# electronicarts/mesh2splat

Measured on AMD Instinct MI355X. Metric: Gaussians/sec emitted (mesh->3DGS conversion pass, density 1024^2), higher is better.
Workload: dtype f32

## Files before the change

include/m2s.h:

```cpp
#ifndef M2S_H
#define M2S_H

#include <stddef.h>
#include <stdint.h>

#ifdef __cplusplus
extern "C" {
#endif

#define M2S_ABI_VERSION 1

typedef enum m2s_status {
    M2S_OK = 0,
    M2S_ERR_INVALID = 1,
    M2S_ERR_NO_DEVICE = 2,
    M2S_ERR_HIP = 3,
    M2S_ERR_OOM = 4,
    M2S_ERR_CAPACITY = 5,
    M2S_ERR_IO = 6,
    M2S_ERR_STATE = 7
} m2s_status;

typedef struct m2s_ctx m2s_ctx;

// ... 290 lines not shown
uint32_t m2s_host_scene_num_meshes(const m2s_host_scene* scene);
const m2s_mesh* m2s_host_scene_meshes(const m2s_host_scene* scene);
const char* m2s_host_scene_mesh_name(const m2s_host_scene* scene, uint32_t i);
const char* m2s_host_scene_warnings(const m2s_host_scene* scene);
m2s_status m2s_read_ply(const char* path, m2s_gaussian** out_records, uint64_t* out_n, int* out_has_pbr);
void m2s_free_records(m2s_gaussian* records);
const char* m2s_io_last_error(void);

enum { M2S_PIPELINE_AUTO = 0, M2S_PIPELINE_MULTIPASS = 1,
       M2S_PIPELINE_TEAM = 3 ,
       M2S_PIPELINE_SPARSE = 4 ,
       M2S_PIPELINE_LEAN = 5  };
m2s_status m2s_set_pipeline(m2s_ctx* ctx, int pipeline);
int m2s_last_pipeline(const m2s_ctx* ctx);
m2s_status m2s_vertex_table(const m2s_ctx* ctx, uint64_t* out_rows, int* out_in_use);

enum { M2S_K_COUNT = 0, M2S_K_SCAN = 1, M2S_K_OFFSETS = 2, M2S_K_EMIT = 3, M2S_K_FUSED = 4, M2S_K_N = 5 };
m2s_status m2s_set_profiling(m2s_ctx* ctx, int enabled);
m2s_status m2s_last_kernel_ms(const m2s_ctx* ctx, float out_ms[M2S_K_N]);
uint64_t m2s_num_triangles(const m2s_ctx* ctx);
m2s_status m2s_debug_set_launch_counter(m2s_ctx* ctx, uint32_t value);

#ifdef __cplusplus
}
#endif
#endif
```

mesh2splat_amd/_lib.py:

```python
from __future__ import annotations

import ctypes as C
import os
import subprocess

_HERE = os.path.dirname(os.path.abspath(__file__))
CSRC = os.path.join(_HERE, "csrc")
LIB_PATH = os.environ.get("M2S_LIB_PATH") or os.path.join(_HERE, "_build", "libm2s_hip.so")

M2S_OK = 0
STATUS_NAMES = {0: "M2S_OK", 1: "M2S_ERR_INVALID", 2: "M2S_ERR_NO_DEVICE", 3: "M2S_ERR_HIP", 4: "M2S_ERR_OOM",
                5: "M2S_ERR_CAPACITY", 6: "M2S_ERR_IO", 7: "M2S_ERR_STATE"}
KERNEL_NAMES = ("count", "scan", "offsets", "emit", "fused")

EXPORTS = (
    "m2s_abi_version", "m2s_create", "m2s_destroy", "m2s_last_error", "m2s_set_triangle_range", "m2s_upload_scene",
    "m2s_set_max_gaussians", "m2s_convert", "m2s_convert_into", "m2s_convert_submit", "m2s_convert_wait", "m2s_last_pipeline", "m2s_set_keep_positions", "m2s_positions_ready", "m2s_debug_set_launch_counter", "m2s_set_async_lanes", "m2s_num_stored", "m2s_device_records", "m2s_download",
    "m2s_download_triangle_counts", "m2s_write_ply", "m2s_export_ply", "m2s_set_profiling", "m2s_last_kernel_ms",
    "m2s_num_triangles", "m2s_set_pipeline", "m2s_load_glb", "m2s_free_host_scene", "m2s_host_scene_num_meshes",
    "m2s_host_scene_meshes", "m2s_host_scene_mesh_name", "m2s_host_scene_warnings", "m2s_read_ply", "m2s_free_records",
    "m2s_io_last_error", "m2s_sort_by_depth", "m2s_device_sorted_records", "m2s_download_sorted", "m2s_last_sort_ms",
    "m2s_upload_records", "m2s_prepass", "m2s_device_quads", "m2s_device_prepass_depths", "m2s_download_prepass", "m2s_last_prepass_ms",
    "m2s_sort_prepass", "m2s_prepass_sorted", "m2s_device_sorted_quads", "m2s_download_sorted_quads", "m2s_last_sort_prepass_ms",
    "m2s_last_upload_ms", "m2s_write_ply_slice", "m2s_export_ply_slice",
# ... 6 lines not shown
    "m2s_last_splat_counts",
    "m2s_shadow", "m2s_shadow_from_quads", "m2s_device_shadow_cubemap", "m2s_download_shadow_cubemap", "m2s_download_shadow_quads", "m2s_upload_shadow_cubemap",
    "m2s_last_shadow_ms", "m2s_last_shadow_stage_ms", "m2s_last_shadow_counts", "m2s_relight", "m2s_upload_gbuffer", "m2s_device_frame",
    "m2s_download_frame", "m2s_download_shadow_counts", "m2s_last_relight_ms",
    "m2s_mesh_depth", "m2s_device_mesh_depth", "m2s_download_mesh_depth", "m2s_last_mesh_depth_ms", "m2s_last_mesh_depth_stage_ms",
    "m2s_last_mesh_depth_counts", "m2s_debug_set_mesh_depth_inplace",
    "m2s_mesh_render", "m2s_device_mesh_gbuffer", "m2s_download_mesh_gbuffer", "m2s_download_mesh_visibility", "m2s_last_mesh_render_ms",
    "m2s_last_mesh_render_stage_ms", "m2s_last_mesh_render_counts", "m2s_relight_split",
    "m2s_relight_mesh", "m2s_device_mesh_frame", "m2s_download_mesh_frame", "m2s_score_frames", "m2s_device_score_map",
    "m2s_download_score_map", "m2s_last_score_ms",
    "m2s_bake_light", "m2s_bake_directions", "m2s_device_sh", "m2s_download_sh", "m2s_download_bake_shadow_counts", "m2s_last_bake_ms",
    "m2s_sh_shade_records", "m2s_write_ply_sh", "m2s_export_ply_sh",
    "m2s_device_sorted_sources", "m2s_download_sorted_sources", "m2s_upload_quad_sources", "m2s_contrib_begin", "m2s_contrib_accumulate", "m2s_device_contrib",
    "m2s_download_contrib", "m2s_last_contrib_ms", "m2s_last_contrib_stage_ms", "m2s_prune", "m2s_last_prune_counts", "m2s_last_prune_ms",
    "m2s_write_ply_compact", "m2s_export_ply_compact", "m2s_last_compact_stage_ms",
    "m2s_vertex_table",
)


class M2SError(RuntimeError):
    def __init__(self, status: int, message: str):
        super().__init__(f"{STATUS_NAMES.get(status, status)}: {message}")
        self.status = status


class Texture(C.Structure):
    _fields_ = [("rgba8", C.c_void_p), ("width", C.c_uint32), ("height", C.c_uint32)]


class MeshC(C.Structure):
    _fields_ = [("vertices", C.c_void_p), ("n_vertices", C.c_uint32), ("stride_floats", C.c_uint32),
# ... 176 lines not shown
        "m2s_download_sorted_sources": (C.c_int, [vp, vp, u64]),
        "m2s_upload_quad_sources": (C.c_int, [vp, vp, u64]),
        "m2s_contrib_begin": (C.c_int, [vp]),
        "m2s_contrib_accumulate": (C.c_int, [vp, vp, C.c_float]),
        "m2s_device_contrib": (vp, [vp, u32]),
        "m2s_download_contrib": (C.c_int, [vp, vp, vp, u64]),
        "m2s_last_contrib_ms": (C.c_float, [vp]),
        "m2s_last_contrib_stage_ms": (C.c_int, [vp, C.POINTER(C.c_float)]),
        "m2s_prune": (C.c_int, [vp, vp, C.POINTER(u64)]),
        "m2s_last_prune_counts": (C.c_int, [vp, C.POINTER(u64)]),
        "m2s_last_prune_ms": (C.c_float, [vp]),
        "m2s_write_ply_compact": (C.c_int, [C.c_char_p, vp, vp, u32, u64, C.c_float, C.POINTER(u64)]),
        "m2s_export_ply_compact": (C.c_int, [vp, C.c_char_p, C.c_float, C.c_int, C.POINTER(u64)]),
        "m2s_last_compact_stage_ms": (C.c_int, [vp, C.POINTER(C.c_float)]),
        "m2s_vertex_table": (C.c_int, [vp, C.POINTER(u64), C.POINTER(C.c_int)]),
    }
    for name, (res, args) in sigs.items():
        fn = getattr(L, name)
        fn.restype = res
        fn.argtypes = args
    _lib = L
    return L
```

mesh2splat_amd/converter.py:

```python
from __future__ import annotations

import ctypes as C
import os
from typing import Optional

import numpy as np

from . import _lib
from .scene import RECORD_FLOATS, TEXTURE_SLOTS, Scene


def marshal_scene(scene: Scene):
    n = scene.n_meshes
    arr = (_lib.MeshC * max(1, n))()
    keep = []
    for i, m in enumerate(scene.meshes):
        v = np.ascontiguousarray(m.vertices, np.float32)
        keep.append(v)
        arr[i].vertices = v.ctypes.data
        arr[i].n_vertices = v.shape[0]
        arr[i].stride_floats = v.shape[1]
        for k in range(3):
            arr[i].bbox_min[k] = float(m.bbox_min[k])
            arr[i].bbox_max[k] = float(m.bbox_max[k])
# ... 754 lines not shown
    def set_pipeline(self, name: str):
        self._check(self._L.m2s_set_pipeline(self._h, {"auto": 0, "multipass": 1, "team": 3, "sparse": 4, "lean": 5}[name]))

    def set_async_lanes(self, lanes: int):
        self._check(self._L.m2s_set_async_lanes(self._h, int(lanes)))

    @property
    def last_pipeline(self) -> str:
        return {0: "none", 1: "multipass", 3: "team", 4: "sparse", 5: "lean"}[self._L.m2s_last_pipeline(self._h)]

    def vertex_table(self) -> dict:
        rows, used = C.c_uint64(0), C.c_int(0)
        self._check(self._L.m2s_vertex_table(self._h, C.byref(rows), C.byref(used)))
        return {"rows": int(rows.value), "in_use": bool(used.value)}

    def set_profiling(self, on: bool):
        self._check(self._L.m2s_set_profiling(self._h, 1 if on else 0))

    def last_kernel_ms(self) -> dict:
        ms = (C.c_float * len(_lib.KERNEL_NAMES))()
        self._check(self._L.m2s_last_kernel_ms(self._h, ms))
        return {k: float(ms[i]) for i, k in enumerate(_lib.KERNEL_NAMES)}


def write_ply(path: str, records: np.ndarray, fmt: int, scale_multiplier: float):
    r = np.ascontiguousarray(records, np.float32)
    if r.ndim != 2 or r.shape[1] != RECORD_FLOATS:
        raise ValueError("records must be (n, 24) float32")
    st = _lib.load().m2s_write_ply(os.fsencode(path), r.ctypes.data, r.shape[0], int(fmt), float(scale_multiplier))
    if st != _lib.M2S_OK:
# ... 140 lines not shown
```

mesh2splat_amd/csrc/m2s_context.cpp:

```cpp
#include "m2s_ctx.h"

#include <algorithm>
#include <chrono>
#include <cstring>
#include <string>

using namespace m2s;
using namespace m2s_host;

namespace {
thread_local std::string g_create_error = "";
}

namespace m2s_host {
void free_scene(m2s_ctx* c) {
    c->tri_mem.release(); c->scene_arena.release();
    c->lane[0].release_scene(false); c->lane[1].release_scene(true);
    c->d_meshes = nullptr; c->d_mesh_first = nullptr;
    c->d_cnt = c->d_partials = nullptr;
    c->d_biglist = nullptr; c->d_bigmeta = nullptr; c->d_bands = nullptr; c->run_table_words = 0; c->d_run_order = nullptr; c->run_order_unit = 0;
    c->d_batch_first = nullptr; c->n_batch_tab = 0; c->chain_words = 0;
    c->rinfo.clear();
    ++c->rinfo_gen;
    c->frag_per_R2 = -1.0;
    c->warm_R = 0; c->warm_total = 0; c->warm_mismatch_seen = false;
    c->sparse_off_R = c->team_off_R = c->lean_off_R = UINT32_MAX;
    c->lean_ok = false;
    c->d_vt_rows.release(); c->d_vt_ids.release();
    c->vt_rows = 0; c->vt_use = false;
    c->scene = SceneDev{};
    c->has_scene = false;
}

m2s_ctx::RInfo& rinfo_for(m2s_ctx* c, uint32_t R) {
    auto it = c->rinfo.find(R);
    if (it != c->rinfo.end()) return it->second;
    if (c->rinfo.size() >= (size_t)kBandSlots) { drain_in_flight(c); c->rinfo.clear(); ++c->rinfo_gen; }
    m2s_ctx::RInfo ri;
    ri.gen = c->rinfo_gen;
    ri.band_slot = (int)c->rinfo.size();
    return c->rinfo.emplace(R, ri).first->second;
}

static bool spin_waits() { static const bool on = !debug_on("M2S_NO_SPIN"); return on; }
// ... 130 lines not shown
        ++c->rinfo_gen;
    }
    c->pipeline = pipeline;
    return M2S_OK;
}

int m2s_last_pipeline(const m2s_ctx* c) { return c ? c->last_pipeline : 0; }

m2s_status m2s_vertex_table(const m2s_ctx* c, uint64_t* out_rows, int* out_in_use) {
    if (!c) return M2S_ERR_INVALID;
    if (out_rows) *out_rows = c->vt_rows;
    if (out_in_use) *out_in_use = c->vt_use ? 1 : 0;
    return M2S_OK;
}

int m2s_positions_ready(const m2s_ctx* c) {
    return c && c->d_pos_plane && c->last_records && c->pos_plane_of == c->last_records && c->pos_plane_n == c->last_stored &&
           c->pos_plane_epoch == c->records_epoch && c->last_stored ? 1 : 0;
}

m2s_status m2s_set_keep_positions(m2s_ctx* c, int enabled) {
    if (!c) return M2S_ERR_INVALID;
    c->keep_positions = enabled != 0;
    return M2S_OK;
}

m2s_status m2s_debug_set_launch_counter(m2s_ctx* c, uint32_t value) {
    if (!c) return M2S_ERR_INVALID;
    if (c->slot_count) return fail(c, M2S_ERR_STATE, kInFlightMsg);
    c->epoch = value;
// ... 19 lines not shown
```

mesh2splat_amd/csrc/m2s_ctx.h:

```cpp
#pragma once
#include "../../include/m2s.h"
#include "m2s_devbuf.h"
#include "m2s_device.h"
#include "m2s_vdedup.h"

#include <cstdint>
#include <cstdlib>
#include <map>
#include <string>

namespace m2s_host {
constexpr uint32_t kMaxGaussiansToSort = 7000000u;
constexpr uint64_t kMaxTriangles = (1ull << 28) - 1;
inline size_t align_up(size_t v, size_t a) { return (v + a - 1) / a * a; }
inline const char* const kStaleMsg = "the records of the conversion last waited for have been overwritten by a later submission at another R "
                                     "(wait for it, or submit into your own buffers)";
inline const char* const kInFlightMsg = "conversions are still in flight: m2s_convert_wait first";
struct GBufPlanes {
    DevBuf<void> plane[5];
    void* ptr[5] = {};
    m2s_status reserve(std::string& err, uint64_t px) {
        for (int k = 0; k < 5; ++k) {
            const m2s_status s = plane[k].reserve(err, px, (k == 2 || k == 4) ? 4 : 8);
            ptr[k] = plane[k].get();
// ... 11 lines not shown
    hipStream_t stream = nullptr;
    std::string err;

    m2s_host::DevBuf<char> tri_mem;
    m2s::SceneDev scene{};
    m2s::MeshParams* d_meshes = nullptr;
    uint32_t* d_mesh_first = nullptr;
    uint32_t n_meshes_total = 0;
    bool has_scene = false;
    bool lean_ok = false;
    uint64_t range_first = 0, range_count = UINT64_MAX;
    m2s_host::DevBuf<float4> d_vt_rows;
    m2s_host::DevBuf<m2s::VtIds> d_vt_ids;
    uint32_t vt_rows = 0;
    bool vt_use = false;

    uint32_t* d_cnt = nullptr;
    uint32_t* d_partials = nullptr;
    m2s_host::PinnedBuf<unsigned long long> h_total;
    static constexpr int kPinnedPrepass = 2 + 2 * M2S_MAX_IN_FLIGHT;
    static constexpr int kPinnedSortMM = 4 + 2 * M2S_MAX_IN_FLIGHT;
    static constexpr int kPinnedWords = 6 + 2 * M2S_MAX_IN_FLIGHT;
    m2s::BigItem* d_biglist = nullptr;
    uint32_t* d_bigmeta = nullptr;
    struct RInfo {
        int form = M2S_PIPELINE_AUTO;
        uint32_t tpw = 0;
        bool async_ok = false;
        bool mp_ready = false;
        bool bands_ready = false;
// ... 236 lines not shown
```

mesh2splat_amd/csrc/m2s_devfn.h:

```cpp
#pragma once
#include "m2s_device.h"
#include "m2s_exact.h"
#include "m2s_vtable.h"

#pragma clang fp contract(off)

namespace m2s {

__device__ __forceinline__ float len3(float x, float y, float z) { return sqrtf((x * x + y * y) + z * z); }
__device__ __forceinline__ float len3sq(float x, float y, float z) { return (x * x + y * y) + z * z; }
__device__ __forceinline__ float inv_len3(float x, float y, float z) {
    const float q = len3sq(x, y, z);
    if (wave_all(in_sqrt_range(q))) return rcp_rn(sqrt_rn(q));
    return 1.0f / sqrtf(q);
}

__device__ __forceinline__ uint32_t wave_incl_scan(uint32_t v, int ) {
    v += (uint32_t)__builtin_amdgcn_update_dpp(0, (int)v, 0x111, 0xf, 0xf, true);
    v += (uint32_t)__builtin_amdgcn_update_dpp(0, (int)v, 0x112, 0xf, 0xf, true);
    v += (uint32_t)__builtin_amdgcn_update_dpp(0, (int)v, 0x114, 0xf, 0xf, true);
    v += (uint32_t)__builtin_amdgcn_update_dpp(0, (int)v, 0x118, 0xf, 0xf, true);
    v += (uint32_t)__builtin_amdgcn_update_dpp(0, (int)v, 0x142, 0xa, 0xf, true);
    v += (uint32_t)__builtin_amdgcn_update_dpp(0, (int)v, 0x143, 0xc, 0xf, true);
    return v;
// ... 576 lines not shown
    float4 rot;
    uint32_t vid_lo, vid_hi;
    uint32_t org;
    uint32_t mesh;
};
static_assert(sizeof(TriShadeSI) == 64, "TriShadeSI must be four float4");
template <class TS> inline constexpr bool kTsHasIds = false;
template <> inline constexpr bool kTsHasIds<TriShadeSI> = true;

__device__ __forceinline__ float lod_from_grad(float fw, float fh, float dudx, float dvdx, float dudy, float dvdy) {
    const float sx = dudx * fw, tx = dvdx * fh, sy = dudy * fw, ty = dvdy * fh;
    const float r2 = fmaxf(fma_(tx, tx, sx * sx), fma_(ty, ty, sy * sy));
    return 0.5f * fast_log2(r2);
}

template <class MP, class TS>
__device__ __forceinline__ void tri_shade_rest(const float p[9], const Geo& g, int a1, int b1, int a2, int b2, MP mp,
                                               float4 b0, float2 b1uv, TS& ts) {
    ts.mesh = 0;
    const float A1 = (float)a1 * 256.0f * ts.inva, B1 = (float)b1 * 256.0f * ts.inva;
    const float A2 = (float)a2 * 256.0f * ts.inva, B2 = (float)b2 * 256.0f * ts.inva;
    geo_flat(p, g, ts.sx, ts.sy, ts.rot);
    ts.lod0 = ts.lod1 = ts.lod2 = 0.0f;
    const auto ta = &mp->tex[0];
    const auto tn = &mp->tex[1];
    const auto tm = &mp->tex[2];
    const bool hasA = ta->texels != nullptr, hasN = tn->texels != nullptr, hasM = tm->texels != nullptr;
    if (hasA || hasN || hasM) {
        const float du1 = b0.z - b0.x, du2 = b1uv.x - b0.x, dv1 = b0.w - b0.y, dv2 = b1uv.y - b0.y;
        const float dudx = fma_(A2, du2, A1 * du1), dvdx = fma_(A2, dv2, A1 * dv1);
        const float dudy = fma_(B2, du2, B1 * du1), dvdy = fma_(B2, dv2, B1 * dv1);
        if (hasA) ts.lod0 = lod_from_grad((float)ta->w, (float)ta->h, dudx, dvdx, dudy, dvdy);
        if (hasN) ts.lod1 = (hasA && tn->w == ta->w && tn->h == ta->h) ? ts.lod0
                          : lod_from_grad((float)tn->w, (float)tn->h, dudx, dvdx, dudy, dvdy);
        if (hasM) ts.lod2 = (hasA && tm->w == ta->w && tm->h == ta->h) ? ts.lod0
                          : (hasN && tm->w == tn->w && tm->h == tn->h) ? ts.lod1
                          : lod_from_grad((float)tm->w, (float)tm->h, dudx, dvdx, dudy, dvdy);
// ... 20 lines not shown
template <class MP>
__device__ __forceinline__ void tri_shade_setup(const float p[9], const Geo& g, const Raster& rs, MP mp,
                                                float4 b0, float2 b1, TriShade& ts) {
    {
#pragma clang fp contract(off)
        ts.inva = rcp_rn((float)rs.area2);
    }
    const long long Px0 = 256ll * rs.x0 + 128, Py0 = 256ll * rs.y0 + 128;
    ts.a1 = rs.a[1]; ts.b1 = rs.b[1]; ts.a2 = rs.a[2]; ts.b2 = rs.b[2];
    ts.e1 = (long long)rs.a[1] * Px0 + (long long)rs.b[1] * Py0 + rs.c[1];
    ts.e2 = (long long)rs.a[2] * Px0 + (long long)rs.b[2] * Py0 + rs.c[2];
    ts.org = ((uint32_t)rs.y0 << 12) | (uint32_t)rs.x0;
    tri_shade_rest(p, g, rs.a[1], rs.b[1], rs.a[2], rs.b[2], mp, b0, b1, ts);
}

template <class MP>
__device__ __forceinline__ void tri_shade_small(const float p[9], const Geo& g, const RasterHead& h, const RasterSmall& rs, MP mp, float4 b0, float2 b1,
                                                uint32_t m, TriShadeS& c) {
    {
#pragma clang fp contract(off)
        c.inva = rcp_rn((float)rs.area2);
    }
    c.a1 = (short)rs.a[1]; c.b1 = (short)rs.b[1]; c.a2 = (short)rs.a[2]; c.b2 = (short)rs.b[2];
    c.e1 = rs.e[1]; c.e2 = rs.e[2];
    c.org = ((uint32_t)h.y0 << 12) | (uint32_t)h.x0;
    tri_shade_rest(p, g, rs.a[1], rs.b[1], rs.a[2], rs.b[2], mp, b0, b1, c);
    c.mesh |= m;
}

struct TexTap {
    uint32_t o00, o10, o01, o11;
    float w00, w10, w01, w11;
};

__device__ __forceinline__ void tex_tap(uint32_t W, uint32_t H, uint32_t level_off, float uf, float vf, TexTap& t) {
    float up, vp;
    {
#pragma clang fp contract(off)
        up = uf * (float)W - 0.5f;
        vp = vf * (float)H - 0.5f;
    }
// ... 321 lines not shown
```

mesh2splat_amd/csrc/m2s_device.h:

```cpp
#pragma once
#include <cstdlib>
#include <hip/hip_runtime.h>
#include <stdint.h>

#include "m2s_vtable.h"

namespace m2s {

#ifdef M2S_DEBUG_BUILD
inline const char* debug_env(const char* name) {
    static const bool enabled = std::getenv("M2S_DEBUG") != nullptr;
    return enabled ? std::getenv(name) : nullptr;
}
#else
inline const char* debug_env(const char*) { return nullptr; }
#endif
inline bool debug_on(const char* name) { const char* v = debug_env(name); return v && *v && *v != '0'; }

constexpr int kBlock = 256;
constexpr int kTriPerBlock = 1024;
constexpr int kEmitF = 1024;
constexpr int kRowsThread = 32;
constexpr int kRowsCount = 128;
constexpr int kStageStride = 7;
// ... 93 lines not shown
    if (const char* v = debug_env("M2S_RUN_SHIFT")) { const uint32_t s = (uint32_t)std::atoi(v) & 15u; return n_units >= (32u << s) ? s : 0u; }
    for (uint32_t shift = 5; shift >= 3; --shift)
        if (n_units >= (32u << shift)) return shift;
    return 0u;
}
inline uint32_t n_runs(uint32_t n_units, uint32_t shift) { return (n_units + (1u << shift) - 1u) >> shift; }
struct BatchTable {
    const uint32_t* first;
    uint32_t n;
    uint32_t tpw;
};
uint32_t fused2_band_workgroups(uint32_t n_tri);
void launch_fused2(const SceneDev& sc, uint32_t R, unsigned long long* chain, uint64_t limit, float4* out,
                   unsigned long long* total, uint32_t* status, uint32_t epoch, BigItem* biglist, uint32_t* bigmeta,
                   const RunInfo& runs, const BatchTable& batches, hipStream_t st);
void launch_fused3(const SceneDev& sc, uint32_t R, unsigned long long* chain, uint64_t limit, float4* out,
                   unsigned long long* total, uint32_t* status, uint32_t epoch, BigItem* biglist, uint32_t* bigmeta,
                   const RunInfo& runs, const BatchTable& batches, hipStream_t st, const VtxTable* vt = nullptr);
void launch_sparse(const SceneDev& sc, uint32_t R, unsigned long long* chain, uint64_t limit, float4* out,
                   unsigned long long* total, uint32_t* status, uint32_t epoch, BigItem* biglist, uint32_t* bigmeta,
                   const RunInfo& runs, hipStream_t st, float4* plane = nullptr);
bool sparse_supported(uint32_t n_tri);
uint32_t sparse_workgroups(uint32_t n_tri);
constexpr uint32_t kSparseTrianglesPerWorkgroup = 512;
void launch_emit_big(const SceneDev& sc, uint32_t R, const BigItem* biglist, uint32_t n_big, uint32_t max_cnt, uint64_t limit,
                     float4* out, hipStream_t st);

struct PrepassK {
    float M[16], V[16], P[16];
    float MinvT[16];
    float mr_inv[9];
    float ms2[3];
    float res[2], near_far[2], std_dev;
// ... 167 lines not shown
```

mesh2splat_amd/csrc/m2s_fused3.hip:

```cpp
#include "m2s_fused_common.h"

#include <type_traits>

#pragma clang fp contract(off)

namespace m2s {

#ifndef M2S_FUSED3_WAVES
#define M2S_FUSED3_WAVES 4
#endif
#ifndef M2S_FUSED3_ENTRIES
#define M2S_FUSED3_ENTRIES 1024
#endif
#ifndef M2S_FUSED3_STAGE
#define M2S_FUSED3_STAGE (M2S_FUSED3_WAVES >= 5 ? 16 : 32)
#endif
constexpr int kL3Team = 4;
constexpr int kL3Threads = kL3Team * 64;
constexpr uint32_t kL3Entries = (uint32_t)M2S_FUSED3_ENTRIES * kL3Team;
constexpr int kL3Stage = M2S_FUSED3_STAGE;
constexpr uint32_t kL3Wait = 1u << 24;
constexpr uint32_t kL3Stop = 1u << 28;

struct F3Ctl {
// ... 76 lines not shown
    return true;
}

#ifdef M2S_TIMELINE
__device__ unsigned long long g_tl_f3[16384 * 4 * 8];
constexpr int kTlHwId = 4 | (31 << 11);
constexpr int kTlXccId = 20 | (3 << 11);
#define TLF(k) do { __builtin_amdgcn_sched_barrier(0); if (lane == 0 && blockIdx.x < 16384u) g_tl_f3[((size_t)blockIdx.x * 4 + wave) * 8 + (k)] = wall_clock64(); __builtin_amdgcn_sched_barrier(0); } while (0)
#define TLFV(k, v) do { if (lane == 0 && blockIdx.x < 16384u) g_tl_f3[((size_t)blockIdx.x * 4 + wave) * 8 + (k)] = (v); } while (0)
#else
#define TLF(k) do { } while (0)
#define TLFV(k, v) do { } while (0)
#endif

struct VtNone { };
template <bool kIndexed>
__global__ void __launch_bounds__(kL3Threads, M2S_FUSED3_WAVES) k_fused3(SceneDev sc, uint32_t R, unsigned long long* __restrict__ chain,
                                                      unsigned long long limit, float4* __restrict__ out,
                                                      unsigned long long* __restrict__ total_out,
                                                      uint32_t* __restrict__ status , uint32_t epoch,
                                                      BigItem* __restrict__ biglist, uint32_t* __restrict__ bigmeta,
                                                      uint32_t tpw ,
                                                      RunInfo runs, BatchTable bt,
                                                      std::conditional_t<kIndexed, VtxTable, VtNone> vt) {
    using TS = std::conditional_t<kIndexed, TriShadeSI, TriShadeS>;
    __shared__ F3Lds S;
    F3Ctl& C = S.ctl;
    const int lane = threadIdx.x & 63;
    const uint32_t wave = __builtin_amdgcn_readfirstlane(threadIdx.x >> 6);
    const uint32_t n_batches = bt.first ? bt.n : (sc.n_tri + tpw - 1u) / tpw;
    const uint32_t hb = blockIdx.x, xcd = hb & 7u, round = hb >> 3;
    const bool in_runs = runs.base != nullptr;
    const uint32_t rmask = (1u << runs.shift) - 1u;
    const unsigned long long etag = (unsigned long long)epoch << kEpochShift;
    uint32_t lb = hb;
    if (in_runs) {
        uint32_t rr = ((round >> runs.shift) << 3) + xcd;
        if (runs.order) rr = ((const __attribute__((address_space(4))) uint32_t*)runs.order)[rr];
        lb = (rr << runs.shift) + (round & rmask);
// ... 25 lines not shown
    const unsigned long long band_base = band_first ? C.base : 0ull;

    uint32_t t0 = b * tpw, nt = tpw;
    if (bt.first && has_batch) {
        const __attribute__((address_space(4))) uint32_t* q = (const __attribute__((address_space(4))) uint32_t*)bt.first;
        t0 = q[b];
        nt = q[b + 1] - t0;
    }
    const uint32_t t = t0 + lane;
    const bool valid = has_batch && (uint32_t)lane < nt && t < sc.n_tri;
    if (lane == 0) C.t0[wave] = t0;
    int kind = kNone;
    unsigned long long mask = 0;
    uint32_t cnt = 0;
    {
        float p[9];
        Geo g;
        RasterHead h;
        h.x0 = h.y0 = 0; h.x1 = h.y1 = -1; h.ext = 0;
        bool box = false;
        uint32_t m = 0;
        float4 uvb0 = make_float4(0, 0, 0, 0);
        float2 uvb1 = make_float2(0, 0);
        [[maybe_unused]] uint2 vid = make_uint2(0, 0);
        bool uniform_mesh = false;
        uint32_t m0 = 0;
        if (has_batch) {
            const uint32_t lastT = min(t0 + nt, sc.n_tri) - 1;
            m0 = mesh_of_range(sc, t0, lastT, uniform_mesh);
            m = m0;
            if (valid) {
                load_positions(sc.tri, t, p);
                uvb0 = sc.tri.B0[t];
                uvb1 = sc.tri.B1[t];
                if constexpr (kIndexed) vid = ld_plane(reinterpret_cast<const uint2*>(vt.ids), t);
                if (uniform_mesh) geo_setup_mp(p, kConstMesh(sc.meshes + m0), g);
                else { m = find_mesh(sc, sc.tri_first + t); geo_setup_mp(p, sc.meshes + m, g); }
                box = raster_head(g, R, h);
            }
        }
        const int w = h.x1 - h.x0 + 1, rows = h.y1 - h.y0 + 1;
        RasterSmall rs;
        bool small = box && w <= 8 && rows <= 8 && h.ext <= 2304;
        if (small) small = raster_small(h, rs);
        else if (box) kind = kBig;
        {
            uint32_t mlo = 0, mhi = 0;
            small_coverage(small, w, rows, rs, mlo, mhi);
            mask = (unsigned long long)mlo | ((unsigned long long)mhi << 32);
            cnt = (uint32_t)__popc(mlo) + (uint32_t)__popc(mhi);
            if (small) kind = kSmall;
        }
        if (cnt != 0 && kind == kSmall) {
            TriShadeS c;
            if (uniform_mesh) tri_shade_small(p, g, h, rs, kConstMesh(sc.meshes + m0), uvb0, uvb1, m, c);
            else tri_shade_small(p, g, h, rs, sc.meshes + m, uvb0, uvb1, m, c);
            const float4* src = reinterpret_cast<const float4*>(&c);
#pragma unroll
            for (int k = 0; k < 3; ++k) S.tri[wave][lane * 4 + k] = src[k];
            if constexpr (kIndexed) S.tri[wave][lane * 4 + 3] = make_float4(__uint_as_float(vid.x), __uint_as_float(vid.y), src[3].z, src[3].w);
            else S.tri[wave][lane * 4 + 3] = src[3];
            float2* const uvs = &S.uv[wave][lane * 3];
            uvs[0] = make_float2(uvb0.x, uvb0.y);
            uvs[1] = make_float2(uvb0.z - uvb0.x, uvb0.w - uvb0.y);
            uvs[2] = make_float2(uvb1.x - uvb0.x, uvb1.y - uvb0.y);
        }
        if (__ballot(kind == kBig) != 0ull) {
            Raster rb;
            rb.x0 = rb.y0 = 0; rb.x1 = rb.y1 = -1; rb.ext = 0; rb.bias = 0; rb.area2 = 1;
#pragma unroll
            for (int i = 0; i < 3; i++) { rb.a[i] = rb.b[i] = 0; rb.c[i] = 0; }
// ... 239 lines not shown
        if (!have_base) have_base = f3_get_base(C, chain, b0, lane, epoch, status, base);
        if (have_base && lane == 0) {
            const unsigned long long out_total = (C.total_w[0] + C.total_w[1]) + (C.total_w[2] + C.total_w[3]);
            chain_store(&chain[b0 + nb_here - 1], kFlagPrefix | etag | ((base + out_total) & kValMask));
            if (b0 + nb_here == n_batches) *total_out = base + out_total;
            if (runs.out && (lb & rmask) == 0u) runs.out[lb >> runs.shift] = base;
        }
    }
    if (err && lane == 0) __hip_atomic_store(&status[1], err, __ATOMIC_RELAXED, __HIP_MEMORY_SCOPE_SYSTEM);
    TLF(5);
    TLFV(7, (unsigned long long)lb | ((unsigned long long)__builtin_amdgcn_s_getreg(kTlHwId) << 32));
}

void launch_fused3(const SceneDev& sc, uint32_t R, unsigned long long* chain, uint64_t limit, float4* out,
                   unsigned long long* total, uint32_t* status, uint32_t epoch, BigItem* biglist, uint32_t* bigmeta,
                   const RunInfo& runs, const BatchTable& bt, hipStream_t st, const VtxTable* vt) {
    const uint32_t tpw = fused_tpw(sc.n_tri);
    const uint32_t n_batches = bt.first ? bt.n : n_fused_waves(sc.n_tri);
    if (!n_batches) return;
    uint32_t nb = (n_batches + kL3Team - 1) / kL3Team;
    RunInfo r = runs;
    if (tpw != 64u || bt.first) r = RunInfo{ nullptr, nullptr, 0u, nullptr };
    if (r.base) r.out = nullptr;
    if (r.base) nb = ((nb + (8u << r.shift) - 1u) / (8u << r.shift)) * (8u << r.shift);
    else nb = (nb + 7u) & ~7u;
    if (vt && vt->rows && vt->ids)
        hipLaunchKernelGGL(k_fused3<true>, dim3(nb), dim3(kL3Threads), 0, st, sc, R, chain, (unsigned long long)limit, out, total, status,
                           epoch & 0xFFFFu, biglist, bigmeta, tpw, r, bt, *vt);
    else
        hipLaunchKernelGGL(k_fused3<false>, dim3(nb), dim3(kL3Threads), 0, st, sc, R, chain, (unsigned long long)limit, out, total, status,
                           epoch & 0xFFFFu, biglist, bigmeta, tpw, r, bt, VtNone{});
}

#ifdef M2S_TIMELINE
}
extern "C" int m2s_debug_timeline_f3(void* dst, size_t bytes) {
    return hipMemcpyFromSymbol(dst, HIP_SYMBOL(m2s::g_tl_f3), std::min(bytes, sizeof(m2s::g_tl_f3))) == hipSuccess ? 0 : 1;
}
extern "C" int m2s_debug_timeline_f3_clear() {
    void* p = nullptr;
    if (hipGetSymbolAddress(&p, HIP_SYMBOL(m2s::g_tl_f3)) != hipSuccess) return 1;
    return hipMemset(p, 0, sizeof(m2s::g_tl_f3)) == hipSuccess ? 0 : 2;
}
namespace m2s {
#endif
uint32_t fused3_resident_workgroups() { return resident_workgroups(reinterpret_cast<const void*>(&k_fused3<false>), kL3Threads); }
hipError_t preload_fused3() { hipFuncAttributes a; return hipFuncGetAttributes(&a, reinterpret_cast<const void*>(&k_fused3<false>)); }

}
```

mesh2splat_amd/csrc/m2s_pass.cpp:

```cpp
#include "m2s_ctx.h"

#include <algorithm>
#include <cstdio>
#include <cstring>
#include <vector>

using namespace m2s;
using namespace m2s_host;

namespace {
static double sparse_frags_per_triangle(uint32_t n_tri) { return n_tri >= 2000000u ? 1.75 : 0.5; }
static uint32_t band_workgroups(const m2s_ctx* c, uint32_t unit) {
    const uint32_t team = fused2_band_workgroups(c->scene.n_tri);
    return !team ? 0u : unit == 256u ? team : sparse_workgroups(c->scene.n_tri);
}
static uint32_t first_resident_slots([[maybe_unused]] int form, [[maybe_unused]] uint32_t shift) {
#ifdef M2S_RUN_ORDER_SPREAD
    const uint32_t wgs = form == M2S_PIPELINE_SPARSE ? sparse_resident_workgroups() : form == M2S_PIPELINE_LEAN ? fused3_resident_workgroups()
                                                                                                                 : fused2_resident_workgroups();
    return wgs >> shift;
#else
    return 0u;
#endif
}
// ... 18 lines not shown
}

BatchTable batches_for(const m2s_ctx* c, const m2s_ctx::RInfo& ri) {
    return c->n_batch_tab ? BatchTable{ c->d_batch_first, c->n_batch_tab, 0u } : BatchTable{ nullptr, 0u, ri.tpw };
}

uint32_t unit_of(int form) { return form == M2S_PIPELINE_SPARSE ? kSparseTrianglesPerWorkgroup : 256u; }

void launch_single(const m2s_ctx* c, const m2s_ctx::RInfo& ri, uint32_t R, unsigned long long* chain, uint64_t limit, float4* d_out,
                   unsigned long long* res, uint32_t epoch, const RunInfo& runs, hipStream_t st, float4* plane) {
    uint32_t* status = reinterpret_cast<uint32_t*>(&res[1]);
    if (ri.form == M2S_PIPELINE_SPARSE)
        launch_sparse(c->scene, R, chain, limit, d_out, &res[0], status, epoch, c->d_biglist, c->d_bigmeta, runs, st, plane);
    else if (ri.form == M2S_PIPELINE_LEAN) {
        const VtxTable vt{ c->d_vt_rows.get(), c->d_vt_ids.get() };
        launch_fused3(c->scene, R, chain, limit, d_out, &res[0], status, epoch, c->d_biglist, c->d_bigmeta, runs, batches_for(c, ri), st,
                      c->vt_use ? &vt : nullptr);
    }
    else
        launch_fused2(c->scene, R, chain, limit, d_out, &res[0], status, epoch, c->d_biglist, c->d_bigmeta, runs, batches_for(c, ri), st);
}

uint64_t resolve_cap(const m2s_ctx* c, uint32_t R) {
    if (c->cap_policy == 0) return 0;
    if (c->cap_policy > 0) return (uint64_t)c->cap_policy;
    const uint32_t mc = std::max<uint32_t>(1u, c->n_meshes_total);
    const uint32_t mx = R * R * 6u * mc;
    return std::min(mx, kMaxGaussiansToSort);
}
}

static bool lean_eligible(const m2s_ctx* c, uint32_t R) {
// ... 402 lines not shown
```

mesh2splat_amd/csrc/m2s_upload.cpp:

```cpp
#include "m2s_ctx.h"
#include "m2s_ply.h"

#include <algorithm>
#include <array>
#include <chrono>
#include <cstring>
#include <thread>
#include <tuple>
#include <vector>

using namespace m2s;
using namespace m2s_host;

namespace {
constexpr size_t kStageChunk = 16ull << 20;

void par_memcpy(void* dst, const void* src, size_t n) {
    const size_t kMin = 2ull << 20;
    unsigned nt = (unsigned)std::min<size_t>(4, n / kMin);
    if (const char* e = std::getenv("M2S_HOST_THREADS")) { if (std::atol(e) == 1) nt = 1; }
    if (nt <= 1) { memcpy(dst, src, n); return; }
    std::vector<std::thread> pool;
    for (unsigned i = 1; i < nt; ++i) {
        const size_t b = n * i / nt, e = n * (i + 1) / nt;
// ... 220 lines not shown
    c->d_batch_first = (uint32_t*)(A + o_batch);
    c->n_batch_tab = 0;
    c->chain_words = chain_words;
    HIPCHK(c, hipMemsetAsync(c->lane[0].chain, 0, chain_words * sizeof(unsigned long long), c->stream));
    HIPCHK(c, hipMemsetAsync(c->d_bigmeta, 0, 4 * sizeof(uint32_t), c->stream));
    const uint32_t warm_R = c->hint_R ? c->hint_R : c->last_R ? c->last_R : 1024u;
    const bool warm = !debug_on("M2S_NO_WARM");
    bool counted = false;
    if (warm && !debug_on("M2S_NO_WARM_OVERLAP")) counted = warm_count_enqueue(c, warm_R) == M2S_OK;
    VtWork vt_work;
    bool vt_begun = false;
    if (vt_size_ok(c->lean_ok, n_tri) && !debug_on("M2S_NO_VTABLE")) {
        vt_begun = vt_dedup_begin(tp, n_tri, vt_work, c->stream) == hipSuccess;
        if (!vt_begun) (void)hipGetLastError();
    }

    for (TexPlan& p : tex_plan) {
        uint32_t* mem = (uint32_t*)(A + p.arena_off);
        const m2s_status st = staged_h2d(c, (const char*)p.src, (size_t)p.d.w * p.d.h * 4, kStageChunk, (char*)mem, turn,
                                         [](char*, size_t, size_t) {});
        if (st != M2S_OK) return st;
        for (uint32_t l = 1; l < p.d.n_levels; ++l)
            launch_mip_level(mem + p.d.off[l - 1], std::max(1u, p.d.w >> (l - 1)), std::max(1u, p.d.h >> (l - 1)),
                             mem + p.d.off[l], std::max(1u, p.d.w >> l), std::max(1u, p.d.h >> l), c->stream);
    }
    for (ComboPlan& cp : combo_plan) {
        uint32_t* mem = (uint32_t*)(A + cp.arena_off);
        const TexDesc &ta = tex_plan[cp.ia].d, &tn = tex_plan[cp.in].d, &tm = tex_plan[cp.im].d;
        for (uint32_t l = 0; l < ta.n_levels; ++l)
            launch_combo_level(ta.texels + ta.off[l], tn.texels + tn.off[l], tm.texels + tm.off[l], std::max(1u, ta.w >> l),
// ... 54 lines not shown
```

Measured before the change: 28.92 billion.

## Precompute per-triangle geometry planes at upload for the lean fused kernel

A new kernel runs at scene upload and computes each triangle's flat-geometry terms (rotation, scales, projected UV offsets), storing them in three float4 planes. The lean fused3 kernel gains a template variant that reads these planes instead of loading positions and running geo_setup and geo_flat on every convert. This moves per-triangle setup work out of the timed conversion pass. In exchange it adds 48 bytes per triangle of device memory and extra loads per triangle in the hot kernel.

```diff
diff --git a/include/m2s.h b/include/m2s.h
--- a/include/m2s.h
+++ b/include/m2s.h
@@ -328,6 +328,7 @@
 m2s_status m2s_set_pipeline(m2s_ctx* ctx, int pipeline);
 int m2s_last_pipeline(const m2s_ctx* ctx);
 m2s_status m2s_vertex_table(const m2s_ctx* ctx, uint64_t* out_rows, int* out_in_use);
+m2s_status m2s_geo_planes(const m2s_ctx* ctx, uint64_t* out_bytes, int* out_in_use);
 
 enum { M2S_K_COUNT = 0, M2S_K_SCAN = 1, M2S_K_OFFSETS = 2, M2S_K_EMIT = 3, M2S_K_FUSED = 4, M2S_K_N = 5 };
 m2s_status m2s_set_profiling(m2s_ctx* ctx, int enabled);
diff --git a/mesh2splat_amd/_lib.py b/mesh2splat_amd/_lib.py
--- a/mesh2splat_amd/_lib.py
+++ b/mesh2splat_amd/_lib.py
@@ -44,7 +44,7 @@
     "m2s_device_sorted_sources", "m2s_download_sorted_sources", "m2s_upload_quad_sources", "m2s_contrib_begin", "m2s_contrib_accumulate", "m2s_device_contrib",
     "m2s_download_contrib", "m2s_last_contrib_ms", "m2s_last_contrib_stage_ms", "m2s_prune", "m2s_last_prune_counts", "m2s_last_prune_ms",
     "m2s_write_ply_compact", "m2s_export_ply_compact", "m2s_last_compact_stage_ms",
-    "m2s_vertex_table",
+    "m2s_vertex_table", "m2s_geo_planes",
 )
 
 
@@ -251,6 +251,7 @@
         "m2s_export_ply_compact": (C.c_int, [vp, C.c_char_p, C.c_float, C.c_int, C.POINTER(u64)]),
         "m2s_last_compact_stage_ms": (C.c_int, [vp, C.POINTER(C.c_float)]),
         "m2s_vertex_table": (C.c_int, [vp, C.POINTER(u64), C.POINTER(C.c_int)]),
+        "m2s_geo_planes": (C.c_int, [vp, C.POINTER(u64), C.POINTER(C.c_int)]),
     }
     for name, (res, args) in sigs.items():
         fn = getattr(L, name)
diff --git a/mesh2splat_amd/converter.py b/mesh2splat_amd/converter.py
--- a/mesh2splat_amd/converter.py
+++ b/mesh2splat_amd/converter.py
@@ -792,6 +792,11 @@
         self._check(self._L.m2s_vertex_table(self._h, C.byref(rows), C.byref(used)))
         return {"rows": int(rows.value), "in_use": bool(used.value)}
 
+    def geo_planes(self) -> dict:
+        nbytes, used = C.c_uint64(0), C.c_int(0)
+        self._check(self._L.m2s_geo_planes(self._h, C.byref(nbytes), C.byref(used)))
+        return {"bytes": int(nbytes.value), "in_use": bool(used.value)}
+
     def set_profiling(self, on: bool):
         self._check(self._L.m2s_set_profiling(self._h, 1 if on else 0))
 
diff --git a/mesh2splat_amd/csrc/m2s_context.cpp b/mesh2splat_amd/csrc/m2s_context.cpp
--- a/mesh2splat_amd/csrc/m2s_context.cpp
+++ b/mesh2splat_amd/csrc/m2s_context.cpp
@@ -28,6 +28,7 @@
     c->lean_ok = false;
     c->d_vt_rows.release(); c->d_vt_ids.release();
     c->vt_rows = 0; c->vt_use = false;
+    c->geo_stride = 0; c->geo_use = false;
     c->scene = SceneDev{};
     c->has_scene = false;
 }
@@ -188,6 +189,13 @@
     return M2S_OK;
 }
 
+m2s_status m2s_geo_planes(const m2s_ctx* c, uint64_t* out_bytes, int* out_in_use) {
+    if (!c) return M2S_ERR_INVALID;
+    if (out_bytes) *out_bytes = c->geo_use ? (uint64_t)c->scene.n_tri * 3u * sizeof(float4) : 0u;
+    if (out_in_use) *out_in_use = c->geo_use ? 1 : 0;
+    return M2S_OK;
+}
+
 int m2s_positions_ready(const m2s_ctx* c) {
     return c && c->d_pos_plane && c->last_records && c->pos_plane_of == c->last_records && c->pos_plane_n == c->last_stored &&
            c->pos_plane_epoch == c->records_epoch && c->last_stored ? 1 : 0;
diff --git a/mesh2splat_amd/csrc/m2s_ctx.h b/mesh2splat_amd/csrc/m2s_ctx.h
--- a/mesh2splat_amd/csrc/m2s_ctx.h
+++ b/mesh2splat_amd/csrc/m2s_ctx.h
@@ -49,6 +49,9 @@
     m2s_host::DevBuf<m2s::VtIds> d_vt_ids;
     uint32_t vt_rows = 0;
     bool vt_use = false;
+    m2s_host::DevBuf<float4> d_geo;
+    size_t geo_stride = 0;
+    bool geo_use = false;
 
     uint32_t* d_cnt = nullptr;
     uint32_t* d_partials = nullptr;
diff --git a/mesh2splat_amd/csrc/m2s_devfn.h b/mesh2splat_amd/csrc/m2s_devfn.h
--- a/mesh2splat_amd/csrc/m2s_devfn.h
+++ b/mesh2splat_amd/csrc/m2s_devfn.h
@@ -614,13 +614,13 @@
     return 0.5f * fast_log2(r2);
 }
 
-template <class MP, class TS>
+template <bool kFlat = true, class MP, class TS>
 __device__ __forceinline__ void tri_shade_rest(const float p[9], const Geo& g, int a1, int b1, int a2, int b2, MP mp,
                                                float4 b0, float2 b1uv, TS& ts) {
     ts.mesh = 0;
     const float A1 = (float)a1 * 256.0f * ts.inva, B1 = (float)b1 * 256.0f * ts.inva;
     const float A2 = (float)a2 * 256.0f * ts.inva, B2 = (float)b2 * 256.0f * ts.inva;
-    geo_flat(p, g, ts.sx, ts.sy, ts.rot);
+    if constexpr (kFlat) geo_flat(p, g, ts.sx, ts.sy, ts.rot);
     ts.lod0 = ts.lod1 = ts.lod2 = 0.0f;
     const auto ta = &mp->tex[0];
     const auto tn = &mp->tex[1];
@@ -671,7 +671,7 @@
     tri_shade_rest(p, g, rs.a[1], rs.b[1], rs.a[2], rs.b[2], mp, b0, b1, ts);
 }
 
-template <class MP>
+template <bool kFlat = true, class MP>
 __device__ __forceinline__ void tri_shade_small(const float p[9], const Geo& g, const RasterHead& h, const RasterSmall& rs, MP mp, float4 b0, float2 b1,
                                                 uint32_t m, TriShadeS& c) {
     {
@@ -681,7 +681,7 @@
     c.a1 = (short)rs.a[1]; c.b1 = (short)rs.b[1]; c.a2 = (short)rs.a[2]; c.b2 = (short)rs.b[2];
     c.e1 = rs.e[1]; c.e2 = rs.e[2];
     c.org = ((uint32_t)h.y0 << 12) | (uint32_t)h.x0;
-    tri_shade_rest(p, g, rs.a[1], rs.b[1], rs.a[2], rs.b[2], mp, b0, b1, c);
+    tri_shade_rest<kFlat>(p, g, rs.a[1], rs.b[1], rs.a[2], rs.b[2], mp, b0, b1, c);
     c.mesh |= m;
 }
 
diff --git a/mesh2splat_amd/csrc/m2s_device.h b/mesh2splat_amd/csrc/m2s_device.h
--- a/mesh2splat_amd/csrc/m2s_device.h
+++ b/mesh2splat_amd/csrc/m2s_device.h
@@ -131,9 +131,16 @@
 void launch_fused2(const SceneDev& sc, uint32_t R, unsigned long long* chain, uint64_t limit, float4* out,
                    unsigned long long* total, uint32_t* status, uint32_t epoch, BigItem* biglist, uint32_t* bigmeta,
                    const RunInfo& runs, const BatchTable& batches, hipStream_t st);
+struct GeoPlanes {
+    const float4* G0;
+    const float4* G1;
+    const float4* G2;
+};
+void launch_geo_planes(const SceneDev& sc, float4* g0, float4* g1, float4* g2, hipStream_t st);
 void launch_fused3(const SceneDev& sc, uint32_t R, unsigned long long* chain, uint64_t limit, float4* out,
                    unsigned long long* total, uint32_t* status, uint32_t epoch, BigItem* biglist, uint32_t* bigmeta,
-                   const RunInfo& runs, const BatchTable& batches, hipStream_t st, const VtxTable* vt = nullptr);
+                   const RunInfo& runs, const BatchTable& batches, hipStream_t st, const VtxTable* vt = nullptr,
+                   const GeoPlanes* gp = nullptr);
 void launch_sparse(const SceneDev& sc, uint32_t R, unsigned long long* chain, uint64_t limit, float4* out,
                    unsigned long long* total, uint32_t* status, uint32_t epoch, BigItem* biglist, uint32_t* bigmeta,
                    const RunInfo& runs, hipStream_t st, float4* plane = nullptr);
diff --git a/mesh2splat_amd/csrc/m2s_fused3.hip b/mesh2splat_amd/csrc/m2s_fused3.hip
--- a/mesh2splat_amd/csrc/m2s_fused3.hip
+++ b/mesh2splat_amd/csrc/m2s_fused3.hip
@@ -114,7 +114,8 @@
 #endif
 
 struct VtNone { };
-template <bool kIndexed>
+struct GeoNone { };
+template <bool kIndexed, bool kGeo>
 __global__ void __launch_bounds__(kL3Threads, M2S_FUSED3_WAVES) k_fused3(SceneDev sc, uint32_t R, unsigned long long* __restrict__ chain,
                                                       unsigned long long limit, float4* __restrict__ out,
                                                       unsigned long long* __restrict__ total_out,
@@ -122,7 +123,8 @@
                                                       BigItem* __restrict__ biglist, uint32_t* __restrict__ bigmeta,
                                                       uint32_t tpw ,
                                                       RunInfo runs, BatchTable bt,
-                                                      std::conditional_t<kIndexed, VtxTable, VtNone> vt) {
+                                                      std::conditional_t<kIndexed, VtxTable, VtNone> vt,
+                                                      std::conditional_t<kGeo, GeoPlanes, GeoNone> gp) {
     using TS = std::conditional_t<kIndexed, TriShadeSI, TriShadeS>;
     __shared__ F3Lds S;
     F3Ctl& C = S.ctl;
@@ -178,8 +180,10 @@
     unsigned long long mask = 0;
     uint32_t cnt = 0;
     {
-        float p[9];
+        [[maybe_unused]] float p[9];
         Geo g;
+        [[maybe_unused]] float4 grot = make_float4(0, 0, 0, 0);
+        [[maybe_unused]] float gsx = 0, gsy = 0;
         RasterHead h;
         h.x0 = h.y0 = 0; h.x1 = h.y1 = -1; h.ext = 0;
         bool box = false;
@@ -194,11 +198,18 @@
             m0 = mesh_of_range(sc, t0, lastT, uniform_mesh);
             m = m0;
             if (valid) {
-                load_positions(sc.tri, t, p);
+                [[maybe_unused]] float4 q0, q1, q2;
+                if constexpr (kGeo) { q0 = ld_plane(gp.G0, t); q1 = ld_plane(gp.G1, t); q2 = ld_plane(gp.G2, t); }
+                else load_positions(sc.tri, t, p);
                 uvb0 = sc.tri.B0[t];
                 uvb1 = sc.tri.B1[t];
                 if constexpr (kIndexed) vid = ld_plane(reinterpret_cast<const uint2*>(vt.ids), t);
-                if (uniform_mesh) geo_setup_mp(p, kConstMesh(sc.meshes + m0), g);
+                if constexpr (kGeo) {
+                    grot = q0; gsx = q1.x; gsy = q1.y;
+                    g.ou[0] = q1.z; g.ov[0] = q1.w; g.ou[1] = q2.x; g.ov[1] = q2.y; g.ou[2] = q2.z; g.ov[2] = q2.w;
+                    if (!uniform_mesh) m = find_mesh(sc, sc.tri_first + t);
+                }
+                else if (uniform_mesh) geo_setup_mp(p, kConstMesh(sc.meshes + m0), g);
                 else { m = find_mesh(sc, sc.tri_first + t); geo_setup_mp(p, sc.meshes + m, g); }
                 box = raster_head(g, R, h);
             }
@@ -217,8 +228,9 @@
         }
         if (cnt != 0 && kind == kSmall) {
             TriShadeS c;
-            if (uniform_mesh) tri_shade_small(p, g, h, rs, kConstMesh(sc.meshes + m0), uvb0, uvb1, m, c);
-            else tri_shade_small(p, g, h, rs, sc.meshes + m, uvb0, uvb1, m, c);
+            if (uniform_mesh) tri_shade_small<!kGeo>(p, g, h, rs, kConstMesh(sc.meshes + m0), uvb0, uvb1, m, c);
+            else tri_shade_small<!kGeo>(p, g, h, rs, sc.meshes + m, uvb0, uvb1, m, c);
+            if constexpr (kGeo) { c.sx = gsx; c.sy = gsy; c.rot = grot; }
             const float4* src = reinterpret_cast<const float4*>(&c);
 #pragma unroll
             for (int k = 0; k < 3; ++k) S.tri[wave][lane * 4 + k] = src[k];
@@ -488,7 +500,7 @@
 
 void launch_fused3(const SceneDev& sc, uint32_t R, unsigned long long* chain, uint64_t limit, float4* out,
                    unsigned long long* total, uint32_t* status, uint32_t epoch, BigItem* biglist, uint32_t* bigmeta,
-                   const RunInfo& runs, const BatchTable& bt, hipStream_t st, const VtxTable* vt) {
+                   const RunInfo& runs, const BatchTable& bt, hipStream_t st, const VtxTable* vt, const GeoPlanes* gp) {
     const uint32_t tpw = fused_tpw(sc.n_tri);
     const uint32_t n_batches = bt.first ? bt.n : n_fused_waves(sc.n_tri);
     if (!n_batches) return;
@@ -498,12 +510,15 @@
     if (r.base) r.out = nullptr;
     if (r.base) nb = ((nb + (8u << r.shift) - 1u) / (8u << r.shift)) * (8u << r.shift);
     else nb = (nb + 7u) & ~7u;
-    if (vt && vt->rows && vt->ids)
-        hipLaunchKernelGGL(k_fused3<true>, dim3(nb), dim3(kL3Threads), 0, st, sc, R, chain, (unsigned long long)limit, out, total, status,
-                           epoch & 0xFFFFu, biglist, bigmeta, tpw, r, bt, *vt);
-    else
-        hipLaunchKernelGGL(k_fused3<false>, dim3(nb), dim3(kL3Threads), 0, st, sc, R, chain, (unsigned long long)limit, out, total, status,
-                           epoch & 0xFFFFu, biglist, bigmeta, tpw, r, bt, VtNone{});
+    const bool indexed = vt && vt->rows && vt->ids, geo = gp && gp->G0 && gp->G1 && gp->G2;
+    auto go = [&](auto kernel, auto table, auto planes) {
+        hipLaunchKernelGGL(kernel, dim3(nb), dim3(kL3Threads), 0, st, sc, R, chain, (unsigned long long)limit, out, total, status,
+                           epoch & 0xFFFFu, biglist, bigmeta, tpw, r, bt, table, planes);
+    };
+    if (indexed && geo) go(k_fused3<true, true>, *vt, *gp);
+    else if (indexed) go(k_fused3<true, false>, *vt, GeoNone{});
+    else if (geo) go(k_fused3<false, true>, VtNone{}, *gp);
+    else go(k_fused3<false, false>, VtNone{}, GeoNone{});
 }
 
 #ifdef M2S_TIMELINE
@@ -518,7 +533,7 @@
 }
 namespace m2s {
 #endif
-uint32_t fused3_resident_workgroups() { return resident_workgroups(reinterpret_cast<const void*>(&k_fused3<false>), kL3Threads); }
-hipError_t preload_fused3() { hipFuncAttributes a; return hipFuncGetAttributes(&a, reinterpret_cast<const void*>(&k_fused3<false>)); }
-
-}
+uint32_t fused3_resident_workgroups() { return resident_workgroups(reinterpret_cast<const void*>(&k_fused3<false, false>), kL3Threads); }
+hipError_t preload_fused3() { hipFuncAttributes a; return hipFuncGetAttributes(&a, reinterpret_cast<const void*>(&k_fused3<false, false>)); }
+
+}
diff --git a/mesh2splat_amd/csrc/m2s_geoplanes.hip b/mesh2splat_amd/csrc/m2s_geoplanes.hip
--- /dev/null
+++ b/mesh2splat_amd/csrc/m2s_geoplanes.hip
@@ -0,0 +1,32 @@
+#include "m2s_device.h"
+#include "m2s_devfn.h"
+
+#pragma clang fp contract(off)
+
+namespace m2s {
+
+__global__ void __launch_bounds__(kBlock) k_geo_planes(SceneDev sc, float4* __restrict__ g0, float4* __restrict__ g1, float4* __restrict__ g2) {
+    const uint32_t wave0 = (blockIdx.x * (uint32_t)kBlock + (threadIdx.x & ~63u));
+    if (wave0 >= sc.n_tri) return;
+    const uint32_t t = wave0 + (threadIdx.x & 63u);
+    bool uniform_mesh = false;
+    const uint32_t m0 = mesh_of_range(sc, wave0, min(wave0 + 64u, sc.n_tri) - 1u, uniform_mesh);
+    if (t >= sc.n_tri) return;
+    float p[9];
+    Geo g;
+    load_positions(sc.tri, t, p);
+    if (uniform_mesh) geo_setup_mp(p, kConstMesh(sc.meshes + m0), g);
+    else geo_setup_mp(p, sc.meshes + find_mesh(sc, sc.tri_first + t), g);
+    float sx, sy;
+    float4 rot;
+    geo_flat(p, g, sx, sy, rot);
+    g0[t] = rot;
+    g1[t] = make_float4(sx, sy, g.ou[0], g.ov[0]);
+    g2[t] = make_float4(g.ou[1], g.ov[1], g.ou[2], g.ov[2]);
+}
+
+void launch_geo_planes(const SceneDev& sc, float4* g0, float4* g1, float4* g2, hipStream_t st) {
+    if (sc.n_tri) hipLaunchKernelGGL(k_geo_planes, dim3((sc.n_tri + kBlock - 1) / kBlock), dim3(kBlock), 0, st, sc, g0, g1, g2);
+}
+
+}
diff --git a/mesh2splat_amd/csrc/m2s_pass.cpp b/mesh2splat_amd/csrc/m2s_pass.cpp
--- a/mesh2splat_amd/csrc/m2s_pass.cpp
+++ b/mesh2splat_amd/csrc/m2s_pass.cpp
@@ -56,8 +56,9 @@
         launch_sparse(c->scene, R, chain, limit, d_out, &res[0], status, epoch, c->d_biglist, c->d_bigmeta, runs, st, plane);
     else if (ri.form == M2S_PIPELINE_LEAN) {
         const VtxTable vt{ c->d_vt_rows.get(), c->d_vt_ids.get() };
+        const GeoPlanes gp{ c->d_geo.get(), c->d_geo.get() + c->geo_stride, c->d_geo.get() + 2 * c->geo_stride };
         launch_fused3(c->scene, R, chain, limit, d_out, &res[0], status, epoch, c->d_biglist, c->d_bigmeta, runs, batches_for(c, ri), st,
-                      c->vt_use ? &vt : nullptr);
+                      c->vt_use ? &vt : nullptr, c->geo_use ? &gp : nullptr);
     }
     else
         launch_fused2(c->scene, R, chain, limit, d_out, &res[0], status, epoch, c->d_biglist, c->d_bigmeta, runs, batches_for(c, ri), st);
diff --git a/mesh2splat_amd/csrc/m2s_upload.cpp b/mesh2splat_amd/csrc/m2s_upload.cpp
--- a/mesh2splat_amd/csrc/m2s_upload.cpp
+++ b/mesh2splat_amd/csrc/m2s_upload.cpp
@@ -258,6 +258,15 @@
         vt_begun = vt_dedup_begin(tp, n_tri, vt_work, c->stream) == hipSuccess;
         if (!vt_begun) (void)hipGetLastError();
     }
+    if (vt_size_ok(c->lean_ok, n_tri) && !debug_on("M2S_NO_GEOPLANES")) {
+        const size_t stride = align_up((size_t)n_tri * sizeof(float4), 256) / sizeof(float4);
+        if (c->d_geo.try_reserve(3 * stride, sizeof(float4))) {
+            launch_geo_planes(c->scene, c->d_geo.get(), c->d_geo.get() + stride, c->d_geo.get() + 2 * stride, c->stream);
+            c->geo_stride = stride;
+            c->geo_use = true;
+        }
+    }
+    if (!c->geo_use) c->d_geo.release();
 
     for (TexPlan& p : tex_plan) {
         uint32_t* mem = (uint32_t*)(A + p.arena_off);
diff --git a/profiles/r11/disassembly_diff.py b/profiles/r11/disassembly_diff.py
--- /dev/null
+++ b/profiles/r11/disassembly_diff.py
@@ -0,0 +1,34 @@
+import re, sys, collections
+def funcs(path):
+    out = collections.OrderedDict()
+    cur = None
+    for line in open(path):
+        m = re.match(r'^(_Z\w+|\w+):\s*(;.*)?$', line)
+        if m and not line.startswith('.L'):
+            cur = m.group(1); out[cur] = []; continue
+        if cur is None: continue
+        s = line.strip()
+        if s.startswith('.Lfunc_end'):
+            cur = None; continue
+        if not s or s.startswith(';') or s.startswith('.') and not s.startswith('.LBB'): continue
+        s = re.sub(r'\s*;.*$', '', s)
+        out[cur].append(s)
+    return out
+def norm(name):
+    m = re.match(r'_ZN3m2s8k_fused3I(Lb[01]E)(Lb0E)?EEvNS_8SceneDev', name)
+    return 'k_fused3<%s>' % m.group(1) if m else name
+PARENT, CAND = sys.argv[1:3]
+for f in sys.argv[3:]:
+    a = funcs('%s/%s.s' % (PARENT, f)); b = funcs('%s/%s.s' % (CAND, f))
+    bn = {norm(k): (k, v) for k, v in b.items()}; a = collections.OrderedDict((norm(k), (k, v)) for k, v in a.items())
+    print('== %s.hip' % f)
+    for k, (pk, v) in a.items():
+        if k.startswith('__hip_cuid'): continue
+        if k not in bn: print('  %-60s parent only' % k[:60]); continue
+        ck, cv = bn[k]
+        def body(name, lines): return [re.sub(r'\.LBB\d+_', '.LBB_', l.replace(name, 'K')) for l in lines]
+        same = body(pk, v) == body(ck, cv)
+        valu = sum(1 for l in v if l.startswith('v_'))
+        print('  %-60s %6d lines %6d v_*  %s' % (k[:60], len(v), valu, 'IDENTICAL' if same else 'DIFFERS (%d lines in candidate)' % len(cv)))
+    for k, (ck, cv) in bn.items():
+        if k not in a and not k.startswith('__hip_cuid'): print('  %-60s candidate only: %d lines, %d v_*' % (ck[:60], len(cv), sum(1 for l in cv if l.startswith('v_'))))
```

Result: faster. 29.89 billion (median of 6 runs) (+3.3%).
